# rsmedleystevenson/pyamg

Measured on AMD Instinct MI355X. Metric: V-cycle iterations/sec (3D Poisson 500^3 fp64, SA-AMG, chebyshev smoother), higher is better.
Workload: dtype f64; 1 GPU; 3D Poisson 500x500x500 (125.0M dof, nnz 873.5M) CSR fp64, smoothed aggregation (5 levels), Chebyshev degree 2 pre/post smoother, V(1,1), b=rand seed 0; parallelism=single GPU

## Files before the change

pyamg_amd/csrc/kernels.hip:

```cpp
#include "amg_dev.hpp"

namespace amg {

constexpr int WG = 256;
#ifndef AMG_TILE
#define AMG_TILE 2048
#endif
constexpr int TILE = AMG_TILE;

typedef int v4i __attribute__((ext_vector_type(4)));
typedef double v2d __attribute__((ext_vector_type(2)));
__device__ __forceinline__ v4i load_v4i(const int *p)
{
#ifdef AMG_NT_LOADS
    return __builtin_nontemporal_load(reinterpret_cast<const v4i *>(p));
#else
    return *reinterpret_cast<const v4i *>(p);
#endif
}
__device__ __forceinline__ v2d load_v2d(const double *p)
{
#ifdef AMG_NT_LOADS
    return __builtin_nontemporal_load(reinterpret_cast<const v2d *>(p));
#else
// ... 1603 lines not shown
            const v2u mm = stream_load(reinterpret_cast<const v2u *>(static_cast<const unsigned *>(E.mask) + i0));
            m[0] = mm.x; m[1] = mm.y;
        }
#pragma unroll
        for (int r = 0; r < 2; ++r)
            if (m[r] & ((NUB == 8) ? 0x80u : 0x80000000u)) m[r] = 0xFFFFFFFFu;
        if (need_b) {
            const v2d bb = stream_load(reinterpret_cast<const v2d *>(&a.b[i0]));
            bval[0] = bb.x; bval[1] = bb.y;
        }
        if (MODE == SM_MATVEC_ACC) { const v2d pp = *reinterpret_cast<const v2d *>(&a.out[i0]); pre2[0] = pp.x; pre2[1] = pp.y; }
        else if (MODE == SM_POLY_LAST || MODE == SM_JACOBI || MODE == SM_JACOBI_BSR1) {
            const v2d pp = *reinterpret_cast<const v2d *>(&a.v2[i0]); pre2[0] = pp.x; pre2[1] = pp.y;
        }
    }
    bool covered[2] = {live0 && m[0] != 0xFFFFFFFFu, live1 && m[1] != 0xFFFFFFFFu};
#pragma unroll
    for (int r = 0; r < 2; ++r) if (!covered[r]) m[r] = 0;
    if (vi) {
        __syncthreads();
#pragma unroll
        for (int r = 0; r < 2; ++r)
#pragma unroll
            for (int u = 0; u < NUB; ++u) v[r][u] = sdict[(unsigned)(cw[r][u >> 3] >> (8 * (u & 7))) & 0xFFu];
    }
    const double gscale = a.gscale;
    double acc[2], diag[2] = {0.0, 0.0};
#pragma unroll
    for (int r = 0; r < 2; ++r) {
        acc[r] = MT::sub ? bval[r] : 0.0;
#pragma unroll
        for (int u = 0; u < NUB; ++u) {
            if (u < E.nu && ((m[r] >> u) & 1u)) {
                if (MT::jac && u == E.u0) { diag[r] = v[r][u]; continue; }
                const double pr = v[r][u] * (gscale * xv[r][u]);
                acc[r] = MT::sub ? (acc[r] - pr) : (acc[r] + pr);
            }
        }
    }

    double res[2] = {0.0, 0.0};
    if (MODE == SM_RESIDUAL_SUMSQ) {
        double sq[2] = {0.0, 0.0};
#pragma unroll
        for (int r = 0; r < 2; ++r)
            if (covered[r]) { res[r] = bval[r] - acc[r]; sq[r] = res[r] * res[r]; }
        if (a.out) {
            if (covered[0] && covered[1]) __builtin_nontemporal_store(v2d{res[0], res[1]}, reinterpret_cast<v2d *>(&a.out[i0]));
            else { if (covered[0]) store_out(&a.out[i0], res[0]); if (covered[1]) store_out(&a.out[i0 + 1], res[1]); }
        }
        *reinterpret_cast<v2d *>(&red[2 * t]) = v2d{sq[0], sq[1]};
        __syncthreads();
        double s0 = red[t], s1 = red[t + WG2];
        for (int off = 32; off > 0; off >>= 1) { s0 += __shfl_down(s0, off, 64); s1 += __shfl_down(s1, off, 64); }
        __syncthreads();
        if ((t & 63) == 0) { red[WG + (t >> 6)] = s0; red[WG + 2 + (t >> 6)] = s1; }
        __syncthreads();
        if (t == 0) {
            double tot = 0.0;
            for (int k = 0; k < 4; ++k) tot += red[WG + k];
            a.out2[blk - E.blk_lo] = tot;
        }
        return;
    }
    bool wr[2] = {covered[0], covered[1]};
#pragma unroll
    for (int r = 0; r < 2; ++r) {
        if (MODE == SM_MATVEC) res[r] = acc[r];
        else if (MODE == SM_MATVEC_ACC) res[r] = pre2[r] + acc[r];
        else if (MODE == SM_RESIDUAL) res[r] = bval[r] - acc[r];
        else if (MODE == SM_POLY_STEP) { const double cr = a.c0 * bval[r]; res[r] = cr + acc[r]; }
        else if (MODE == SM_POLY_LAST) { const double cr = a.c0 * bval[r]; const double h = cr + acc[r]; res[r] = pre2[r] + h; }
        else if (MODE == SM_JACOBI) {
            if (diag[r] != 0.0) { const double q = (bval[r] - acc[r]) / diag[r]; const double t1 = (1.0 - a.c0) * pre2[r]; const double t2 = a.c0 * q; res[r] = t1 + t2; }
            else res[r] = pre2[r];
        } else if (MODE == SM_JACOBI_BSR1) {
            if (diag[r] != 0.0) { const double t1 = (1.0 - a.c0) * pre2[r]; const double t2 = (a.c0 * acc[r]) / diag[r]; res[r] = t1 + t2; }
            else res[r] = pre2[r];
        }
    }
    constexpr bool streamed = (MODE == SM_MATVEC || MODE == SM_MATVEC_ACC || MODE == SM_RESIDUAL || MODE == SM_POLY_LAST);
    if (wr[0] && wr[1]) {
        if (streamed) __builtin_nontemporal_store(v2d{res[0], res[1]}, reinterpret_cast<v2d *>(&a.out[i0]));
        else *reinterpret_cast<v2d *>(&a.out[i0]) = v2d{res[0], res[1]};
    } else {
        if (wr[0]) { if (streamed) store_out(&a.out[i0], res[0]); else a.out[i0] = res[0]; }
        if (wr[1]) { if (streamed) store_out(&a.out[i0 + 1], res[1]); else a.out[i0 + 1] = res[1]; }
    }
    (void)both;
}

static int g_stencil_coded = std::getenv("AMG_STENCIL_CODED") ? std::atoi(std::getenv("AMG_STENCIL_CODED")) : 1;
static int g_stencil_pairs = 1;
void set_stencil_pairs(int on) { g_stencil_pairs = on; ++g_config_epoch; }

struct StencilRanges { int n; int range[STENCIL_RANGES][2]; };

__global__ void stencil_build_kernel(int n, const int *Ap, const double *Ax, const int *pat, const int *dict_ptr,
                                     const int *dict_slot, const unsigned *pat_mask, int nu, double *vals,
                                     void *mask, StencilRanges R)
{
    const int i = blockIdx.x * blockDim.x + threadIdx.x;
    if (i >= n) return;
    const int p = pat[i];
    unsigned pm = pat_mask[p];
    for (int r = 0; r < R.n; ++r)
        if (i >= R.range[r][0] && i < R.range[r][1]) pm = 0x80000000u;
    if (nu <= 7) static_cast<unsigned char *>(mask)[i] = (pm & 0x80000000u) ? (unsigned char)0x80 : (unsigned char)pm;
    else static_cast<unsigned *>(mask)[i] = pm;
    if (pm & 0x80000000u) return;
    const int s = Ap[i], e = Ap[i + 1], d = dict_ptr[p];
    double *vp = vals + ((size_t)(i / WG) * nu) * WG + (i % WG);
    for (int k = s; k < e; ++k) vp[(size_t)dict_slot[d + (k - s)] * WG] = Ax[k];
}

int launch_stencil_build(const DevCsr &M, const int *dict_slot, const unsigned *pat_mask, hipStream_t st)
{
    const int n = M.nrows;
    StencilRanges R;
    R.n = M.st_nranges;
    for (int r = 0; r < STENCIL_RANGES; ++r) { R.range[r][0] = M.st_range[r][0]; R.range[r][1] = M.st_range[r][1]; }
    hipLaunchKernelGGL(stencil_build_kernel, dim3((n + 255) / 256), dim3(256), 0, st, n, M.Ap, M.Ax, M.pat,
                       M.dict_ptr, dict_slot, pat_mask, M.st_nu, M.st_vals, M.st_mask, R);
    hipError_t e = hipGetLastError();
    if (e != hipSuccess) return hip_fail(e, "stencil build launch", __FILE__, __LINE__);
    return 0;
}

__global__ void value_scan_kernel(const double *vals, long count, unsigned long long *table, int *overflow)
{
    const unsigned long long EMPTY = ~0ULL;
    for (long k = blockIdx.x * (long)blockDim.x + threadIdx.x; k < count; k += (long)gridDim.x * blockDim.x) {
        const unsigned long long bits = (unsigned long long)__double_as_longlong(vals[k]);
        if (bits == EMPTY) { *overflow = 1; continue; }
        unsigned h = (unsigned)((bits * 0x9E3779B97F4A7C15ULL) >> 54);
        bool done = false;
        for (int probe = 0; probe < 1024 && !done; ++probe, h = (h + 1) & 1023u) {
            unsigned long long cur = table[h];
            if (cur == bits) { done = true; break; }
            if (cur == EMPTY) {
                cur = atomicCAS(&table[h], EMPTY, bits);
                if (cur == EMPTY || cur == bits) { done = true; break; }
            }
        }
        if (!done) *overflow = 1;
    }
}
__global__ void value_encode_kernel(const double *vals, long count, const double *dict, int ndict, unsigned char *codes,
                                    int nu, const unsigned char *mask8, long nrows)
{
    const int nw = (nu + 7) >> 3;
    for (long k = blockIdx.x * (long)blockDim.x + threadIdx.x; k < count; k += (long)gridDim.x * blockDim.x) {
        const long long bits = __double_as_longlong(vals[k]);
        int lo = 0, hi = ndict - 1, at = 0;
        while (lo <= hi) {
            const int mid = (lo + hi) >> 1;
            const long long d = __double_as_longlong(dict[mid]);
            if (d == bits) { at = mid; break; }
            if (d < bits) lo = mid + 1; else hi = mid - 1;
        }
        const long blk = k / ((long)nu * WG);
        const int rem = (int)(k - blk * (long)nu * WG);
        const int slot = rem / WG, t = rem - slot * WG;
        if (mask8) {
            const long row = blk * WG + t;
            const unsigned m = row < nrows ? mask8[row] : 0u;
            if ((m & 0x80u) || !((m >> slot) & 1u)) at = 255;
        }
        codes[((blk * nw + (slot >> 3)) * WG + t) * 8 + (slot & 7)] = (unsigned char)at;
    }
}
int launch_value_scan(const double *vals, long count, unsigned long long *table, int *overflow, hipStream_t st)
{
    hipLaunchKernelGGL(value_scan_kernel, dim3(8192), dim3(256), 0, st, vals, count, table, overflow);
    hipError_t e = hipGetLastError();
    if (e != hipSuccess) return hip_fail(e, "value scan launch", __FILE__, __LINE__);
    return 0;
}
int launch_value_encode(const double *vals, long count, const double *dict_sorted, int ndict, unsigned char *codes, int nu,
                        hipStream_t st, const unsigned char *mask8, long nrows)
{
    hipLaunchKernelGGL(value_encode_kernel, dim3(8192), dim3(256), 0, st, vals, count, dict_sorted, ndict, codes, nu, mask8, nrows);
    hipError_t e = hipGetLastError();
    if (e != hipSuccess) return hip_fail(e, "value encode launch", __FILE__, __LINE__);
    return 0;
}

static int g_stencil_form = 1;
void set_stencil_form(int on) { g_stencil_form = on; ++g_config_epoch; }
bool stencil_enabled() { return g_stencil_form != 0; }

static int stencil_own_blocks(const StreamArgs &a)
{
    if (a.row_hi <= a.row_lo) return 0;
    return (a.row_hi - 1) / WG - a.row_lo / WG + 1;
}

static int pattern_rpb(const StreamArgs &a)
{
    int rpb = a.rows_per_wg;
    if (rpb < 1 || rpb > WG) rpb = WG;
    return rpb;
}

int stencil_blocks(const StreamArgs &a, const DevCsr &M)
{
    int nb = stencil_own_blocks(a);
    const int rpb = pattern_rpb(a);
    for (int r = 0; r < M.st_nranges; ++r) {
        const int lo = std::max(a.row_lo, M.st_range[r][0]), hi = std::min(a.row_hi, M.st_range[r][1]);
        if (hi > lo) nb += (hi - lo + rpb - 1) / rpb;
    }
    return nb;
}

template <int MODE>
static int launch_stencil_mode(const StreamArgs &a, const DevCsr &M, hipStream_t st)
{
    const int nb = stencil_own_blocks(a);
    if (nb <= 0) return 0;
    StreamArgs b = a;
    if (b.gscale == 0.0) b.gscale = 1.0;
    StencilArgs E;
    E.vals = M.st_vals; E.mask = M.st_mask; E.nu = M.st_nu; E.u0 = M.st_u0;
    E.codes = (M.st_vi_on && M.st_codes) ? M.st_codes : nullptr; E.dict = M.st_dict; E.ndict = M.st_ndict;
    E.ranges = M.st_nranges;
    E.blk_lo = a.row_lo / WG; E.nblocks = nb; E.ncols = M.ncols;
    E.period_blocks = E.seg_blocks = 0;
    for (int u = 0; u < STENCIL_MAX; ++u) E.off[u] = M.st_off[u];
    int grid = nb;
    if (g_xcd_period && M.period_rows > 0) {
        const int S = (M.period_rows + WG / 2) / WG;
        const int G = (S + 7) / 8;
        if (S >= 64 && nb >= 4 * S && 3.0 * G * WG * 8.0 <= 2.0e6) {
            E.period_blocks = S;
            E.seg_blocks = G;
            grid = 8 * G * ((nb + S - 1) / S);
        }
    }
    const bool big = (long)(a.row_hi - a.row_lo) >= 30000000L && M.st_nu <= 7;
    static const int pairs_coded = std::getenv("AMG_STENCIL_PAIRS_CODED") ? std::atoi(std::getenv("AMG_STENCIL_PAIRS_CODED")) : 0;
    const bool pairs = (g_stencil_pairs >= 2 || (g_stencil_pairs == 1 && big)) && M.st_nu <= 16 && (E.codes == nullptr || pairs_coded) &&
                       (((uintptr_t)b.b | (uintptr_t)b.out | (uintptr_t)b.v2 | (uintptr_t)b.xg) & 15u) == 0;
    if (pairs && M.st_nu <= 7)
        hipLaunchKernelGGL((stencil2_kernel<MODE, 8>), dim3(grid), dim3(WG2), 0, st, b, E, g_xcd_chunk);
    else if (pairs)
        hipLaunchKernelGGL((stencil2_kernel<MODE, 16>), dim3(grid), dim3(WG2), 0, st, b, E, g_xcd_chunk);
    else if (E.codes != nullptr && M.st_nu <= 7 && g_stencil_coded)
        hipLaunchKernelGGL((stencil_coded_kernel<MODE>), dim3(grid), dim3(WG), 0, st, b, E, g_xcd_chunk);
    else if (M.st_nu <= 7)
        hipLaunchKernelGGL((stencil_kernel<MODE, 8>), dim3(grid), dim3(WG), 0, st, b, E, g_xcd_chunk);
    else if (M.st_nu <= 16)
        hipLaunchKernelGGL((stencil_kernel<MODE, 16>), dim3(grid), dim3(WG), 0, st, b, E, g_xcd_chunk);
    else
        hipLaunchKernelGGL((stencil_kernel<MODE, 32>), dim3(grid), dim3(WG), 0, st, b, E, g_xcd_chunk);
    hipError_t e = hipGetLastError();
    if (e != hipSuccess) return hip_fail(e, "stencil launch", __FILE__, __LINE__);
    const int rpb = pattern_rpb(a);
    int done = nb;
    for (int r = 0; r < M.st_nranges; ++r) {
        StreamArgs c = a;
        c.row_lo = std::max(a.row_lo, M.st_range[r][0]);
        c.row_hi = std::min(a.row_hi, M.st_range[r][1]);
        if (c.row_hi <= c.row_lo) continue;
        if (MODE == SM_RESIDUAL_SUMSQ) c.out2 = a.out2 + done;
        int rc = launch_pattern((StreamMode)MODE, c, M, st);
        if (rc != 0) return rc;
        done += (c.row_hi - c.row_lo + rpb - 1) / rpb;
    }
    return 0;
}

int launch_stencil(StreamMode mode, const StreamArgs &a, const DevCsr &M, hipStream_t st)
{
    switch (mode) {
    case SM_MATVEC: return launch_stencil_mode<SM_MATVEC>(a, M, st);
    case SM_MATVEC_ACC: return launch_stencil_mode<SM_MATVEC_ACC>(a, M, st);
    case SM_RESIDUAL: return launch_stencil_mode<SM_RESIDUAL>(a, M, st);
    case SM_POLY_STEP: return launch_stencil_mode<SM_POLY_STEP>(a, M, st);
    case SM_POLY_LAST: return launch_stencil_mode<SM_POLY_LAST>(a, M, st);
    case SM_JACOBI: return launch_stencil_mode<SM_JACOBI>(a, M, st);
    case SM_JACOBI_BSR1: return launch_stencil_mode<SM_JACOBI_BSR1>(a, M, st);
    case SM_RESIDUAL_SUMSQ: return launch_stencil_mode<SM_RESIDUAL_SUMSQ>(a, M, st);
    default: break;
    }
    set_error("launch_stencil: mode not supported");
    return -1;
}

#ifndef L0C_TY
#define L0C_TY 16
#endif
constexpr int L0C_TX = 32;
constexpr int L0C_WG = L0C_TX * L0C_TY;
constexpr int L0C_PAD = L0C_TX;

template <int FR, int LR>
__global__ __launch_bounds__(L0C_WG) void level0_chain_kernel(Level0ChainArgs a)
{
    constexpr int S = FR + 1 + LR;
    constexpr int SP = FR + 1;
    constexpr int INX = L0C_TX - 2 * S, INY = L0C_TY - 2 * S;
    __shared__ double sdict[256];
    __shared__ double pl[S][L0C_WG + 2 * L0C_PAD];
    const int t = threadIdx.x, tx = t % L0C_TX, ty = t / L0C_TX;
    const int bid = remap_block(blockIdx.x, gridDim.x, 16);
    const int tiles = a.tiles_x * a.tiles_y;
    const int zb = bid / tiles, rem = bid - zb * tiles;
    const int tyi = rem / a.tiles_x, txi = rem - tyi * a.tiles_x;
    const int gx = txi * INX - S + tx, gy = tyi * INY - S + ty;
    const bool inxy = gx >= 0 && gx < a.nx && gy >= 0 && gy < a.ny;
    const bool ring1 = inxy && tx >= 1 && tx < L0C_TX - 1 && ty >= 1 && ty < L0C_TY - 1;
    const bool inner = inxy && tx >= S && tx < L0C_TX - S && ty >= S && ty < L0C_TY - S;
    const long P = (long)a.nx * a.ny;
    const long col = inxy ? (long)gy * a.nx + gx : 0;
    const int z0 = zb * a.zc, z1 = min(z0 + a.zc, a.nz);
    if (t < a.ndict) sdict[t] = a.dict[t];

    double w[S + 1][3];
    unsigned long long cq[S];
    double bq[S];
#pragma unroll
    for (int s = 0; s <= S; ++s) w[s][0] = w[s][1] = w[s][2] = 0.0;
#pragma unroll
    for (int s = 0; s < S; ++s) { cq[s] = ~0ULL; bq[s] = 0.0; }
    double xq = 0.0;
    int k = z0 - S;
    double g_next = (inxy && k >= 0) ? a.g0[(long)k * P + col] : 0.0;
    unsigned long long c_next = ~0ULL;
    double b_next = 0.0, x_next = 0.0;
    const int iters = (z1 - z0) + 2 * S;
    for (int j = 0; j < iters; ++j, ++k) {
        w[0][0] = w[0][1]; w[0][1] = w[0][2]; w[0][2] = g_next;
#pragma unroll
        for (int s = S - 1; s > 0; --s) { cq[s] = cq[s - 1]; bq[s] = bq[s - 1]; }
        cq[0] = c_next; bq[0] = b_next; xq = x_next;
        {
            const int kn = k + 1;
            g_next = (inxy && kn >= 0 && kn < a.nz) ? a.g0[(long)kn * P + col] : 0.0;
            const bool rowk = ring1 && k >= 0 && k < a.nz;
            const long ik = (long)k * P + col;
            c_next = rowk ? a.codes[ik] : ~0ULL;
            b_next = rowk ? a.b[ik] : 0.0;
            if (!FR) x_next = rowk ? a.x[ik] : 0.0;
        }
#pragma unroll
        for (int s = 1; s <= S; ++s) {
            pl[s - 1][L0C_PAD + t] = w[s - 1][1];
            __syncthreads();
            const double *q = &pl[s - 1][L0C_PAD + t];
            const double xv[7] = {w[s - 1][0], q[-L0C_TX], q[-1], w[s - 1][1], q[1], q[L0C_TX], w[s - 1][2]};
            double diag = 0.0, val;
            if (s == SP) {
                const double acc = coded_row_sum<SM_POLY_LAST>(cq[s - 1], sdict, xv, a.c_gs, true, 0.0, -1, diag);
                val = poly_last_row(a.c_last, w[s - 1][1], acc, FR ? w[0][0] : xq);
            } else {
                const double acc = coded_row_sum<SM_RESIDUAL>(cq[s - 1], sdict, xv, 1.0, true, 0.0, -1, diag);
                val = residual_row(bq[s - 1], acc);
            }
            w[s][0] = w[s][1]; w[s][1] = w[s][2]; w[s][2] = val;
        }
        const int p = k - S;
        if (inner && p >= z0 && p < z1) {
            const long i = (long)p * P + col;
            if (LR) store_out(&a.rout[i], w[S][2]);
            store_out(&a.xout[i], w[SP][2 - (S - SP)]);
        }
    }
}

int level0_chain_tile(int stages, int axis) { return (axis == 0 ? L0C_TX : L0C_TY) - 2 * stages; }
int level0_chain_lanes(int axis) { return axis == 0 ? L0C_TX : L0C_TY; }

int launch_level0_chain(bool first_res, bool last_res, const Level0ChainArgs &a0, hipStream_t st)
{
    Level0ChainArgs a = a0;
    const int S = 1 + (first_res ? 1 : 0) + (last_res ? 1 : 0);
    if (S < 2 || a.nx < 1 || a.ny < 1 || a.nz < 1 || a.zc < 1) { set_error("launch_level0_chain: bad chain"); return -1; }
    const int inx = level0_chain_tile(S, 0), iny = level0_chain_tile(S, 1);
    a.tiles_x = (a.nx + inx - 1) / inx;
    a.tiles_y = (a.ny + iny - 1) / iny;
    const long grid = (long)a.tiles_x * a.tiles_y * ((a.nz + a.zc - 1) / a.zc);
    if (grid > 2147483647L) { set_error("launch_level0_chain: grid too large"); return -1; }
    if (first_res && last_res) hipLaunchKernelGGL((level0_chain_kernel<1, 1>), dim3(grid), dim3(L0C_WG), 0, st, a);
    else if (first_res) hipLaunchKernelGGL((level0_chain_kernel<1, 0>), dim3(grid), dim3(L0C_WG), 0, st, a);
    else hipLaunchKernelGGL((level0_chain_kernel<0, 1>), dim3(grid), dim3(L0C_WG), 0, st, a);
    hipError_t e = hipGetLastError();
    if (e != hipSuccess) return hip_fail(e, "level-0 chain launch", __FILE__, __LINE__);
    return 0;
}

constexpr int SSQ_BLOCKS = 8;
__global__ __launch_bounds__(WG) void sumsq_partials_kernel(const double *r, int n, int nb, double *out2)
{
    __shared__ double red[SSQ_BLOCKS][8];
    const int t = threadIdx.x, b0 = blockIdx.x * SSQ_BLOCKS;
    double sq[SSQ_BLOCKS];
#pragma unroll
    for (int q = 0; q < SSQ_BLOCKS; ++q) {
        const long i = (long)(b0 + q) * WG + t;
        sq[q] = 0.0;
        if (i < n) {
            const double rr = r[i];
            sq[q] = rr * rr;
        }
    }
#pragma unroll
    for (int q = 0; q < SSQ_BLOCKS; ++q) {
        const double tot = block_reduce_sum(sq[q], red[q]);
        if (t == 0 && b0 + q < nb) out2[b0 + q] = tot;
    }
}

int launch_sumsq_partials(const double *r, int n, double *out2, hipStream_t st)
{
    if (n <= 0) return 0;
    const int nb = (n + WG - 1) / WG;
    hipLaunchKernelGGL(sumsq_partials_kernel, dim3((nb + SSQ_BLOCKS - 1) / SSQ_BLOCKS), dim3(WG), 0, st, r, n, nb, out2);
    hipError_t e = hipGetLastError();
    if (e != hipSuccess) return hip_fail(e, "sumsq partials launch", __FILE__, __LINE__);
    return 0;
}

__global__ void level0_box_scan_kernel(const unsigned long long *codes, int nx, int ny, int nz, int *bad)
{
    const long n = (long)nx * ny * nz;
    for (long i = blockIdx.x * (long)blockDim.x + threadIdx.x; i < n; i += (long)gridDim.x * blockDim.x) {
        const unsigned long long cw = codes[i];
        const int x = (int)(i % nx);
        const long r = i / nx;
        const int y = (int)(r % ny), z = (int)(r / ny);
        const bool ok[7] = {z > 0, y > 0, x > 0, true, x < nx - 1, y < ny - 1, z < nz - 1};
        bool fail = false;
#pragma unroll
        for (int u = 0; u < 7; ++u) fail |= ((unsigned)(cw >> (8 * u)) & 0xFFu) != 255u && !ok[u];
        if (fail) *bad = 1;
    }
}

int launch_level0_box_scan(const unsigned char *codes, int nx, int ny, int nz, int *bad, hipStream_t st)
{
    hipLaunchKernelGGL(level0_box_scan_kernel, dim3(4096), dim3(256), 0, st, reinterpret_cast<const unsigned long long *>(codes),
                       nx, ny, nz, bad);
    hipError_t e = hipGetLastError();
    if (e != hipSuccess) return hip_fail(e, "level-0 box scan launch", __FILE__, __LINE__);
    return 0;
}

__global__ __launch_bounds__(WG) void index16_build_kernel(int nrows, int rpb, const int *Ap, const int *Aj,
                                                          unsigned short *Aj16, int *wg_base, unsigned char *wg_flag)
{
    __shared__ int sset[16];
    __shared__ int sover;
    const int t = threadIdx.x, wg = blockIdx.x;
    const int r0 = wg * rpb;
    const int nr = min(rpb, nrows - r0);
    const int kbeg = Ap[r0], kend = Ap[r0 + nr];
    if (t < 16) sset[t] = -1;
    if (t == 0) sover = 0;
    __syncthreads();
    for (int k = kbeg + t; k < kend; k += WG) {
        const int w = Aj[k] >> 12;
        bool placed = false;
        for (int s = 0; s < 16 && !placed; ++s) {
            int cur = atomicCAS(&sset[s], -1, w);
            placed = (cur == -1 || cur == w);
        }
        if (!placed) sover = 1;
    }
    __syncthreads();
    if (sover) {
        if (t == 0) wg_flag[wg] = 0;
        return;
    }
    for (int k = kbeg + t; k < kend; k += WG) {
        const int c = Aj[k], w = c >> 12;
        int slot = 0;
        for (int s = 0; s < 16; ++s) if (sset[s] == w) slot = s;
        Aj16[k] = (unsigned short)((slot << 12) | (c & 4095));
    }
    if (t < 16) wg_base[wg * 16 + t] = sset[t] >= 0 ? (sset[t] << 12) : 0;
    if (t == 0) wg_flag[wg] = 1;
}

static int g_index16 = 0;
void set_index16(int on) { g_index16 = on; ++g_config_epoch; }
bool index16_enabled() { return g_index16 != 0; }

int launch_index16_build(DevCsr &M, int rpb, hipStream_t st)
{
    const int nwg = (M.nrows + rpb - 1) / rpb;
    if (nwg <= 0) return 0;
    hipLaunchKernelGGL(index16_build_kernel, dim3(nwg), dim3(WG), 0, st, M.nrows, rpb, M.Ap, M.Aj, M.Aj16, M.wg_base,
                       M.wg_flag);
    hipError_t e = hipGetLastError();
    if (e != hipSuccess) return hip_fail(e, "index16 build launch", __FILE__, __LINE__);
    return 0;
}

template <int MODE>
static int launch_stream_mode(const StreamArgs &a, hipStream_t st)
{
    int rows = a.row_hi - a.row_lo;
    if (rows <= 0) return 0;
    int rpb = a.rows_per_wg;
    if (rpb < 1 || rpb > WG) rpb = WG;
    int nb = (rows + rpb - 1) / rpb;
    StreamArgs b = a;
    if (b.gscale == 0.0) b.gscale = 1.0;
    if (!g_index16 || (a.row_lo % rpb) != 0) b.Aj16 = nullptr;
    if constexpr (!ModeTraits<MODE>::gs) {
        if (g_stream_pipe && g_stream_variant && !b.Aj16) {
            static int per_cu = 0;
            if (per_cu == 0) {
                int nbk = 0;
                if (hipOccupancyMaxActiveBlocksPerMultiprocessor(&nbk, csr_stream_pipe_kernel<MODE>, WG, 0) != hipSuccess || nbk < 1) nbk = 4;
                per_cu = nbk;
            }
            static int ncu = 0;
            if (ncu == 0) {
                int dev = 0; hipDeviceProp_t pr;
                if (hipGetDevice(&dev) == hipSuccess && hipGetDeviceProperties(&pr, dev) == hipSuccess) ncu = pr.multiProcessorCount;
                if (ncu < 8) ncu = 256;
            }
            int G = per_cu * ncu;
            G -= G % 8;
            if (G > nb) G = nb;
            hipLaunchKernelGGL((csr_stream_pipe_kernel<MODE>), dim3(G), dim3(WG), 0, st, b, g_xcd_chunk, rpb, nb);
            hipError_t e = hipGetLastError();
            if (e != hipSuccess) return hip_fail(e, "csr_stream_pipe launch", __FILE__, __LINE__);
            return 0;
        }
    }
    if (g_stream_variant)
        hipLaunchKernelGGL((csr_stream_kernel<MODE, 1>), dim3(nb), dim3(WG), 0, st, b, g_xcd_chunk, rpb);
    else
        hipLaunchKernelGGL((csr_stream_kernel<MODE, 0>), dim3(nb), dim3(WG), 0, st, b, g_xcd_chunk, rpb);
    hipError_t e = hipGetLastError();
    if (e != hipSuccess) return hip_fail(e, "csr_stream launch", __FILE__, __LINE__);
    return 0;
}

constexpr int GS_LEVEL_MAXWG = 224;
struct LevelEntries { int e[GS_LEVEL_MAXWG + 1]; };

template <bool BSR1>
__global__ __launch_bounds__(WG) void gs_level_kernel(StreamArgs a, LevelEntries H, int rpb)
{
    __shared__ double sp[TILE];
    const int t = threadIdx.x;
    const int blk = blockIdx.x;
    const int r0 = a.row_lo + blk * rpb;
    const int nr = min(rpb, a.row_hi - r0);
    const int kbeg = H.e[blk], kend = H.e[blk + 1];
    constexpr int U = TILE / WG;
    int c[U];
    double v[U];
#pragma unroll
    for (int u = 0; u < U; ++u) {
        const int k = kbeg + u * WG + t;
        const bool ok = k < kend;
        c[u] = ok ? a.Aj[k] : 0;
        v[u] = ok ? a.Ax[k] : 0.0;
    }
    int my_s = kend, my_e = kend, row = r0 + t, dpos = -1;
    if (t < nr) {
        my_s = a.Ap[r0 + t];
        my_e = a.Ap[r0 + t + 1];
        if (a.rowmap) row = a.rowmap[r0 + t];
        dpos = a.diagpos[r0 + t];
    }
    double gs_d = 0.0, gs_b = 0.0;
    double acc = 0.0;
    for (int tile_lo = kbeg; tile_lo < kend; tile_lo += TILE) {
        const int tile_hi = min(tile_lo + TILE, kend);
        if (tile_lo != kbeg) {
#pragma unroll
            for (int u = 0; u < U; ++u) {
                const int k = tile_lo + u * WG + t;
                const bool ok = k < tile_hi;
                c[u] = ok ? a.Aj[k] : 0;
                v[u] = ok ? a.Ax[k] : 0.0;
            }
        }
        double xv[U];
#pragma unroll
        for (int u = 0; u < U; ++u) xv[u] = a.xg[c[u]];
        if (tile_lo == kbeg && t < nr) {
            gs_d = (dpos >= 0) ? a.Ax[dpos] : 0.0;
            gs_b = a.b[row];
            if (BSR1) acc = gs_b;
        }
#pragma unroll
        for (int u = 0; u < U; ++u) sp[u * WG + t] = v[u] * xv[u];
        __syncthreads();
        {
            const int s = max(my_s, tile_lo), e2 = min(my_e, tile_hi);
            constexpr int RB = AMG_ROWSUM_BATCH;
            for (int k = s; k < e2; k += RB) {
                double p[RB];
#pragma unroll
                for (int u = 0; u < RB; ++u) p[u] = sp[min(k + u, e2 - 1) - tile_lo];
#pragma unroll
                for (int u = 0; u < RB; ++u) {
                    const bool take = (k + u < e2) && (k + u != dpos);
                    const double nxt = BSR1 ? (acc - p[u]) : (acc + p[u]);
                    acc = take ? nxt : acc;
                }
            }
        }
        __syncthreads();
    }
    if (t >= nr) return;
    if (kbeg >= kend) {
        gs_d = (dpos >= 0) ? a.Ax[dpos] : 0.0;
        gs_b = a.b[row];
        if (BSR1) acc = gs_b;
    }
    if (gs_d != 0.0) a.out[row] = BSR1 ? (acc / gs_d) : ((gs_b - acc) / gs_d);
}

static int g_gs_level_hint = 1;
void set_gs_level_hint(int on) { g_gs_level_hint = on; ++g_config_epoch; }

int launch_gs_level(const StreamArgs &a, bool bsr1, const int *gp_host, hipStream_t st)
{
    const int rows = a.row_hi - a.row_lo;
    if (rows <= 0) return 0;
    int rpb = a.rows_per_wg;
    if (rpb < 1 || rpb > WG) rpb = WG;
    const int nb = (rows + rpb - 1) / rpb;
    if (!gp_host || !g_gs_level_hint || nb > GS_LEVEL_MAXWG || a.Aj16 != nullptr || (a.gscale != 0.0 && a.gscale != 1.0))
        return launch_stream(bsr1 ? SM_GS_BSR1 : SM_GS, a, st);
    LevelEntries H;
    for (int g = 0; g <= nb; ++g) H.e[g] = gp_host[std::min(a.row_lo + g * rpb, a.row_hi)];
    for (int g = nb + 1; g <= GS_LEVEL_MAXWG; ++g) H.e[g] = H.e[nb];
    if (bsr1) hipLaunchKernelGGL((gs_level_kernel<true>), dim3(nb), dim3(WG), 0, st, a, H, rpb);
    else hipLaunchKernelGGL((gs_level_kernel<false>), dim3(nb), dim3(WG), 0, st, a, H, rpb);
    hipError_t e = hipGetLastError();
    if (e != hipSuccess) return hip_fail(e, "gs level launch", __FILE__, __LINE__);
    return 0;
}

int stream_blocks(const StreamArgs &a)
{
    int rows = a.row_hi - a.row_lo;
    int rpb = a.rows_per_wg;
    if (rpb < 1 || rpb > WG) rpb = WG;
    return rows > 0 ? (rows + rpb - 1) / rpb : 0;
}

int launch_stream(StreamMode mode, const StreamArgs &a, hipStream_t st)
{
    switch (mode) {
    case SM_MATVEC: return launch_stream_mode<SM_MATVEC>(a, st);
    case SM_MATVEC_ACC: return launch_stream_mode<SM_MATVEC_ACC>(a, st);
    case SM_RESIDUAL: return launch_stream_mode<SM_RESIDUAL>(a, st);
    case SM_POLY_FIRST: return launch_stream_mode<SM_POLY_FIRST>(a, st);
    case SM_POLY_STEP: return launch_stream_mode<SM_POLY_STEP>(a, st);
    case SM_POLY_LAST: return launch_stream_mode<SM_POLY_LAST>(a, st);
    case SM_JACOBI: return launch_stream_mode<SM_JACOBI>(a, st);
    case SM_JACOBI_BSR1: return launch_stream_mode<SM_JACOBI_BSR1>(a, st);
    case SM_GS: return launch_stream_mode<SM_GS>(a, st);
    case SM_GS_BSR1: return launch_stream_mode<SM_GS_BSR1>(a, st);
    case SM_RESIDUAL_SUMSQ: return launch_stream_mode<SM_RESIDUAL_SUMSQ>(a, st);
    }
    set_error("launch_stream: bad mode");
    return -1;
}

__global__ void jacobi_rows_kernel(const int *Ap, const int *Aj, const double *Ax,
                                   const double *temp, const double *b, double *x, int row_start,
                                   int count, int row_step, double omega)
{
    int t = blockIdx.x * blockDim.x + threadIdx.x;
    if (t >= count) return;
    int i = row_start + t * row_step;
    double rsum = 0.0, diag = 0.0;
    for (int jj = Ap[i]; jj < Ap[i + 1]; ++jj) {
        int j = Aj[jj];
        if (i == j) diag = Ax[jj];
        else rsum = rsum + Ax[jj] * temp[j];
    }
    if (diag != 0.0) {
        double q = (b[i] - rsum) / diag;
        double t1 = (1.0 - omega) * temp[i];
        double t2 = omega * q;
        x[i] = t1 + t2;
    }
}

int launch_jacobi_rows(const DevCsr &A, const double *temp, const double *b, double *x,
                       int row_start, int count, int row_step, double omega, hipStream_t st)
{
    if (count <= 0) return 0;
    hipLaunchKernelGGL(jacobi_rows_kernel, dim3((count + 255) / 256), dim3(256), 0, st, A.Ap, A.Aj,
                       A.Ax, temp, b, x, row_start, count, row_step, omega);
    hipError_t e = hipGetLastError();
    if (e != hipSuccess) return hip_fail(e, "jacobi_rows launch", __FILE__, __LINE__);
    return 0;
}

static inline int vec_grid(long n)
{
    long nb = (n + 255) / 256;
    if (nb > 256L * 16) nb = 256L * 16;
    if (nb < 1) nb = 1;
    return (int)nb;
}

__global__ void scale_kernel(double *out, const double *in, double c, long n)
{
    for (long i = blockIdx.x * (long)blockDim.x + threadIdx.x; i < n; i += (long)gridDim.x * blockDim.x)
        out[i] = c * in[i];
}
__global__ void fill_kernel(double *out, double v, long n)
{
    for (long i = blockIdx.x * (long)blockDim.x + threadIdx.x; i < n; i += (long)gridDim.x * blockDim.x)
        out[i] = v;
}
__global__ void sor_combine_kernel(double *x, const double *xold, double omega, long n)
// ... 537 lines not shown
```

Before: 89.65 V-cycle iterations/s.

## Double-buffer level-0 chain planes with one barrier; wave-level sum-of-squares partials

The level-0 chain kernel now writes all stage planes into a double-buffered shared array indexed by iteration parity and uses a single barrier per z-step instead of one per stage. It stores w[s-1][2] for later stages instead of w[s-1][1], which relies on the stage pipelining matching the earlier per-stage writes. This raises shared memory use to two buffers, which may lower occupancy. Separately, the sum-of-squares partials kernel has each wave reduce whole 256-element chunks with shuffles, removing shared-memory block reductions and their barriers.

```diff
diff --git a/pyamg_amd/csrc/kernels.hip b/pyamg_amd/csrc/kernels.hip
--- a/pyamg_amd/csrc/kernels.hip
+++ b/pyamg_amd/csrc/kernels.hip
@@ -1929,7 +1929,7 @@
     constexpr int SP = FR + 1;
     constexpr int INX = L0C_TX - 2 * S, INY = L0C_TY - 2 * S;
     __shared__ double sdict[256];
-    __shared__ double pl[S][L0C_WG + 2 * L0C_PAD];
+    __shared__ double pl[2][S][L0C_WG + 2 * L0C_PAD];
     const int t = threadIdx.x, tx = t % L0C_TX, ty = t / L0C_TX;
     const int bid = remap_block(blockIdx.x, gridDim.x, 16);
     const int tiles = a.tiles_x * a.tiles_y;
@@ -1971,11 +1971,13 @@
             b_next = rowk ? a.b[ik] : 0.0;
             if (!FR) x_next = rowk ? a.x[ik] : 0.0;
         }
+        double (*plb)[L0C_WG + 2 * L0C_PAD] = pl[j & 1];
+#pragma unroll
+        for (int s = 1; s <= S; ++s) plb[s - 1][L0C_PAD + t] = s == 1 ? w[0][1] : w[s - 1][2];
+        __syncthreads();
 #pragma unroll
         for (int s = 1; s <= S; ++s) {
-            pl[s - 1][L0C_PAD + t] = w[s - 1][1];
-            __syncthreads();
-            const double *q = &pl[s - 1][L0C_PAD + t];
+            const double *q = &plb[s - 1][L0C_PAD + t];
             const double xv[7] = {w[s - 1][0], q[-L0C_TX], q[-1], w[s - 1][1], q[1], q[L0C_TX], w[s - 1][2]};
             double diag = 0.0, val;
             if (s == SP) {
@@ -2017,25 +2019,31 @@
     return 0;
 }
 
-constexpr int SSQ_BLOCKS = 8;
+constexpr int SSQ_BLOCKS = 2;
 __global__ __launch_bounds__(WG) void sumsq_partials_kernel(const double *r, int n, int nb, double *out2)
 {
-    __shared__ double red[SSQ_BLOCKS][8];
-    const int t = threadIdx.x, b0 = blockIdx.x * SSQ_BLOCKS;
-    double sq[SSQ_BLOCKS];
+    static_assert(WG == 256, "a block of the partials is four wave-sized pieces");
+    const int lane = threadIdx.x & 63;
+    const int b0 = (blockIdx.x * (WG / 64) + (threadIdx.x >> 6)) * SSQ_BLOCKS;
+    double sq[SSQ_BLOCKS][4];
+#pragma unroll
+    for (int q = 0; q < SSQ_BLOCKS; ++q)
+#pragma unroll
+        for (int p = 0; p < 4; ++p) {
+            const long i = (long)(b0 + q) * WG + 64 * p + lane;
+            const double rr = i < n ? r[i] : 0.0;
+            sq[q][p] = rr * rr;
+        }
 #pragma unroll
     for (int q = 0; q < SSQ_BLOCKS; ++q) {
-        const long i = (long)(b0 + q) * WG + t;
-        sq[q] = 0.0;
-        if (i < n) {
-            const double rr = r[i];
-            sq[q] = rr * rr;
-        }
-    }
-#pragma unroll
-    for (int q = 0; q < SSQ_BLOCKS; ++q) {
-        const double tot = block_reduce_sum(sq[q], red[q]);
-        if (t == 0 && b0 + q < nb) out2[b0 + q] = tot;
+        double tot = 0.0;
+#pragma unroll
+        for (int p = 0; p < 4; ++p) {
+            double v = sq[q][p];
+            for (int off = 32; off > 0; off >>= 1) v += __shfl_down(v, off, 64);
+            tot += v;
+        }
+        if (lane == 0 && b0 + q < nb) out2[b0 + q] = tot;
     }
 }
 
@@ -2043,7 +2051,8 @@
 {
     if (n <= 0) return 0;
     const int nb = (n + WG - 1) / WG;
-    hipLaunchKernelGGL(sumsq_partials_kernel, dim3((nb + SSQ_BLOCKS - 1) / SSQ_BLOCKS), dim3(WG), 0, st, r, n, nb, out2);
+    const int per_wg = SSQ_BLOCKS * (WG / 64);
+    hipLaunchKernelGGL(sumsq_partials_kernel, dim3((nb + per_wg - 1) / per_wg), dim3(WG), 0, st, r, n, nb, out2);
     hipError_t e = hipGetLastError();
     if (e != hipSuccess) return hip_fail(e, "sumsq partials launch", __FILE__, __LINE__);
     return 0;
```

New measurement: 91.87 V-cycle iterations/s (median of 6 runs). 2.5% higher.
